# pps-lab/rofl-project-code

Measured on AMD Instinct MI355X. Metric: range-proof elements/sec (create+verify), d=25k 32-bit, higher is better.
Workload: dtype u32x8 (255-bit integer field)

## Files before the change

rofl_project_code_amd/csrc/host_msm.hpp:

```cpp
#pragma once

MsmPlan msm_plan(size_t n, size_t np = 1) {
    MsmPlan p;
    static const size_t t13 = knob("ROFL_MSM_T13") ? (size_t)atol(knob("ROFL_MSM_T13")) : ((size_t)1 << 13);
    static const size_t t10_knob = knob("ROFL_MSM_T10") ? (size_t)atol(knob("ROFL_MSM_T10")) : 0;
    const size_t t10 = t10_knob ? t10_knob : (np >= 32 ? (size_t)1 << 11 : (size_t)1 << 9);
    if (n >= (1u << 17)) p.c = 16; else if (n >= t13) p.c = 13; else if (n >= t10) p.c = 10; else if (n >= 64) p.c = 7; else p.c = 4;
    if (const char *e = knob("ROFL_MSM_C")) { int v = atoi(e); if (v == 4 || v == 7 || v == 10 || v == 13 || v == 16) p.c = (u32)v; }
    p.W = (254 + p.c - 1) / p.c;
    p.W = (253 - p.c + p.c - 1) / p.c + 1;
    p.wide = (253 - p.c) - (p.c - 1) * (p.W - 1);
    p.B = 1u << (p.c - 1);
    p.levels = (p.c - 1) / 3;
    return p;
}
struct MsmOpt { u32 lr_nh = 0, lr_ng = 0; const niels *fb_wtab = nullptr; size_t fb_stride = 0; u32 fb_c = 16; std::function<void()> overlap; std::function<void(size_t)> post; u32 tag = 0;
                std::function<void(size_t, int)> post8;
                const sc *ip_dev = nullptr; u32 ip_nblk = 0; const niels *qpts = nullptr; bool *ip_included = nullptr;
                hipEvent_t pts_ready = nullptr; };

struct MsmAllow { bool fb = true, small = true, two = true, slots = true; };
enum class MsmKind { FixedBase, Small, Slots, CountSort };
struct MsmJob {
    MsmWs *ws = nullptr; size_t np = 0, nq = 0, n = 0, PW = 0; MsmPlan P{}; MsmKind kind = MsmKind::CountSort; bool lr = false, two = false, dev_horner = false;
// ... 157 lines not shown
            u32 best = tile; double best_cost = cost(tile);
            for (u32 t = iter_pts; t < n_side + iter_pts; t += iter_pts) {
                const size_t tiles = (n_side + t - 1) / t;
                if (tiles > 48 || tiles * PW > 4096) continue;
                const double c = cost(t);
                if (c < best_cost * 0.999) { best = t; best_cost = c; }
            }
            if (knob("ROFL_TRACE")) fprintf(stderr, "[rofl] bin_l1 tiling: n_side=%u PW=%zu iter=%u: tile %u (%zu blocks, cost %.0f) -> best %u (%zu blocks, cost %.0f)\n", n_side, PW, iter_pts, tile,
                                            (size_t)((n_side + tile - 1) / tile) * PW, cost(tile), best, (size_t)((n_side + best - 1) / best) * PW, best_cost);
            if (best_cost < 0.85 * cost(tile)) tile = best;
        }
        dim3 grid((n_side + tile - 1) / tile, (u32)PW);
        { KSpan ks(C.tm, st, ROFL_TK_MSM_SCATTER, 0, terms * 32 + terms * P.W * 4);
          ROFL_LAUNCH(k_msm_bin_l1, grid, dim3(1024), (size_t)(tl.nbins + tl.nbins * tl.stage) * 4, st, n_side, tile, iter_pts, mw, mm, d_probs, bcur, bins, btail, tl, d_flag);
          ROFL_LAUNCH(k_msm_bin_l2, dim3(tl.nbins, (u32)PW), dim3(512), (size_t)(2 * 128 * worder_wps + tl.cap_bin) * 4, st, tl, P.B, bcur, bins, (const u32 *)btail, cnt, off, d_flag,
                      worder_wps, worder_shift); }
        ROFL_LAUNCH(k_msm_scan, dim3((unsigned)PW), dim3(P.B >= 1024 ? 1024 : 256), 0, st, P.B, cnt, off, (u32 *)nullptr, perm);
        if (C.tm.enabled) { e0 = C.tm.get(); e1 = C.tm.get(); HIPCHK(hipEventRecord(e0, st)); }
        {
            KSpan ks_acc(C.tm, st, ROFL_TK_MSM_ACCUMULATE_FB, terms * P.W * 7, terms * 32);
            static const char *timeline = knob("ROFL_DBG_ACC_TIMELINE");
            if (timeline) {
                dim3 g = grid1((size_t)Wb * P.B, (u32)nq);
                size_t waves = (size_t)g.x * g.y * (TPB / 64);
                unsigned long long *rec; HIPCHK(hipMalloc(&rec, waves * 32)); HIPCHK(hipMemsetAsync(rec, 0, waves * 32, st));
                ROFL_LAUNCH(k_msm_accumulate_fb_dbg, g, dim3(TPB), 0, st, (u32)n, P.c, Wb, (u32)(np / nq), d_probs, cnt, off, bins, perm, buckets, MSM_LIST_ABS, acc_balance, rec);
                std::vector<unsigned long long> h(waves * 4);
                HIPCHK(hipMemcpyAsync(h.data(), rec, waves * 32, hipMemcpyDeviceToHost, st)); HIPCHK(hipStreamSynchronize(st));
                if (FILE *f = fopen(timeline, "ab")) { unsigned long long hdr[4] = {0x54494d45ull, waves, g.x, g.y}; fwrite(hdr, 8, 4, f); fwrite(h.data(), 8, h.size(), f); fclose(f); }
                HIPCHK(hipFree(rec));
            } else
            ROFL_LAUNCH(k_msm_accumulate_fb, grid1((size_t)Wb * P.B, (u32)nq), dim3(TPB), 0, st, (u32)n, P.c, Wb, (u32)(np / nq), d_probs, cnt, off, bins, perm, buckets, MSM_LIST_ABS,
                        acc_balance | ((worder && nq > 1 && Wb > 1) ? 2u : 0u));
        }
        if (C.tm.enabled) HIPCHK(hipEventRecord(e1, st));
    } else if (J.kind != MsmKind::CountSort) {
        HIPCHK(hipMemsetAsync(cnt, 0, sizeof(u32) * (PW * P.B + 4), st));
        const u32 cap = J.cap;
        u32 *slots = W.sorted.as<u32>(PW * P.B * cap);
        MsmOvf *ovf = W.ovf.as<MsmOvf>(MSM_OVF_MAX);
        u32 *ovf_count = cnt + PW * P.B;
        if (C.msm_lds && n >= C.msm_lds_min && (size_t)P.B * 4 <= 128 * 1024) {
            u32 per_q = fb ? J.sets : P.W;
            u32 tile = n_side;
            u32 wps = fb ? mm.fb_wps : 1;
            while (tile > 1024 && ((size_t)tile * wps > (size_t)C.msm_lds_tile || (size_t)((n_side + tile - 1) / tile) * nq * (lr ? 2 : 1) * per_q < 256)) tile /= 2;
            dim3 grid((n_side + tile - 1) / tile, (u32)(nq * (lr ? 2 : 1) * per_q));
            J.tile = tile;
            uint64_t items = terms * P.W;
            KSpan ks(C.tm, st, ROFL_TK_MSM_SCATTER, 0, terms * 32 + items * 4);
            ROFL_LAUNCH(k_msm_scatter_lds, grid, dim3(1024), (size_t)P.B * 4, st, n_side, tile, mw, mm, d_probs, cnt, slots, cap, ovf_count, ovf, MSM_OVF_MAX);
        } else
            ROFL_LAUNCH(k_msm_scatter_slots, grid1(n, (u32)(nq * P.W)), dim3(TPB), 0, st, (u32)n, mw, mm, d_probs, cnt, slots, cap, ovf_count, ovf, MSM_OVF_MAX);
        ROFL_LAUNCH(k_msm_scan, dim3((unsigned)PW), dim3(P.B >= 1024 ? 1024 : 256), 0, st, P.B, cnt, off, (u32 *)nullptr, perm);
        if (opt.pts_ready) HIPCHK(hipStreamWaitEvent(st, opt.pts_ready, 0));
        if (C.tm.enabled) { e0 = C.tm.get(); e1 = C.tm.get(); HIPCHK(hipEventRecord(e0, st)); }
        {
            uint64_t acc_adds = terms * P.W;
            KSpan ks_acc(C.tm, st, fb ? ROFL_TK_MSM_ACCUMULATE_FB : ROFL_TK_MSM_ACCUMULATE_GEN, acc_adds * 7, terms * 32);
            if (fb) ROFL_LAUNCH(k_msm_accumulate_fb, grid1((size_t)Wb * P.B, (u32)nq), dim3(TPB), 0, st, (u32)n, P.c, Wb, (u32)(np / nq), d_probs, cnt, off, slots, perm, buckets, cap, acc_balance);
            else ROFL_LAUNCH(k_msm_accumulate_gen, grid1((size_t)Wb * P.B, (u32)nq), dim3(TPB), 0, st, (u32)n, P.c, Wb, (u32)(np / nq), d_probs, cnt, off, slots, perm, buckets, cap, acc_balance);
        }
        if (C.tm.enabled) HIPCHK(hipEventRecord(e1, st));
        ROFL_LAUNCH(k_msm_overflow, dim3(1), dim3(64), 0, st, Wb, P.B, (u32)(np / nq), d_probs, ovf_count, ovf, MSM_OVF_MAX, buckets, fb ? 1 : 0);
        HIPCHK(hipMemcpyAsync(h_flag, ovf_count, 4, hipMemcpyDeviceToHost, st));
    } else {
        HIPCHK(hipMemsetAsync(cnt, 0, sizeof(u32) * (PW * P.B + 4), st));
        u32 *sorted = W.sorted.as<u32>(PW * n * 2);
        ROFL_LAUNCH(k_msm_count, grid1(n, (u32)(nq * P.W)), dim3(TPB), 0, st, (u32)n, mw, mm, d_probs, cnt);
        ROFL_LAUNCH(k_msm_scan, dim3((unsigned)PW), dim3(P.B >= 1024 ? 1024 : 256), 0, st, P.B, cnt, off, cur, perm);
        ROFL_LAUNCH(k_msm_scatter, grid1(n, (u32)(nq * P.W)), dim3(TPB), 0, st, (u32)n, mw, mm, d_probs, cur, sorted);
        if (opt.pts_ready) HIPCHK(hipStreamWaitEvent(st, opt.pts_ready, 0));
        if (C.tm.enabled) { e0 = C.tm.get(); e1 = C.tm.get(); HIPCHK(hipEventRecord(e0, st)); }
        ROFL_LAUNCH(k_msm_accumulate_gen, grid1((size_t)Wb * P.B, (u32)nq), dim3(TPB), 0, st, (u32)n, P.c, Wb, (u32)(np / nq), d_probs, cnt, off, sorted, perm, buckets, 0u, acc_balance);
        if (C.tm.enabled) HIPCHK(hipEventRecord(e1, st));
    }
    if (C.tm.enabled) {
        C.tm.acc_ev.push_back({e0, e1}); C.tm.t.msm_accumulate_launches++; C.tm.t.msm_additions += terms * P.W;
        char tg[96]; snprintf(tg, sizeof tg, "msm np=%zu n=%zu c=%u cap=%u fb=%u lr=%d", np, n, P.c, J.kind != MsmKind::CountSort ? J.cap : 0u, fb ? J.sets : 0u, (int)lr); C.tm.acc_tag.push_back(tg);
    }
    const ge *S_in = buckets; const ge *C_in = nullptr;
    u32 E = P.B, nb = 0, lv = 0;
    uint64_t red_adds = 0;
    { u32 e = P.B, b = 0; while (e > 512) { red_adds += (uint64_t)(e / 8) * (11 + 7 * b); e /= 8; b += 3; }
      red_adds += (uint64_t)(e / 8) * (16 + 7 * b); e /= 8; b += 3; while (e > 1) { red_adds += (uint64_t)(e / 2) * (1 + b); e /= 2; b++; } }
    ge *S_fin = J.dev_horner ? W.S[1].as<ge>(PW) : hres_dev;
    ge *C_fin = J.dev_horner ? W.Cacc[1].as<ge>(PW * (size_t)nb_final) : hres_dev + PW;
    {
        KSpan ks_red(C.tm, st, ROFL_TK_MSM_REDUCE, red_adds * PW * 9, (uint64_t)PW * P.B * 128);
        while (E > 512) {
            u32 E8 = E / 8;
            ge *S_out = W.S[lv & 1].as<ge>(PW * E8);
            ge *C_out = W.Cacc[lv & 1].as<ge>(PW * (size_t)(nb + 3) * E8);
            ROFL_LAUNCH(k_msm_reduce_level, grid1((size_t)E8 * (1 + nb), (u32)PW), dim3(TPB), 0, st, E, nb, S_in, C_in, S_out, C_out);
            S_in = S_out; C_in = C_out; E = E8; nb += 3; lv++;
        }
        if (J.dev_horner) { S_fin = W.S[lv & 1].as<ge>(PW); C_fin = W.Cacc[lv & 1].as<ge>(PW * (size_t)nb_final); }
        static const u32 red_fused_max = knob("ROFL_RED_FUSED_T") ? (u32)std::max(64, atoi(knob("ROFL_RED_FUSED_T"))) : 768u;
        u32 fused_items = (E / 8) * (4 + nb), fused_threads = fused_items > 512 ? (fused_items > 640 ? 768 : 640) : fused_items > 256 ? 512 : fused_items > 128 ? 256 : fused_items > 64 ? 128 : 64;
        if (fused_threads > red_fused_max) fused_threads = red_fused_max;
        J.fused_t = fused_threads;
        size_t lds = ((size_t)(E / 8) * (1 + nb + 3) + (size_t)(E / 16) * (1 + nb + 4) + 1) * sizeof(ge);
        ROFL_LAUNCH(k_msm_reduce_fused, dim3((unsigned)PW), dim3(fused_threads), lds, st, E, nb, S_in, C_in, S_fin, C_fin, nb_final);
    }
    if (J.host8)
        ROFL_LAUNCH(k_msm_wsum, grid1(PW * 4), dim3(TPB), 0, st, (u32)PW, (const ge *)S_fin, (const ge *)C_fin, nb_final, hres_dev);
    else if (J.dev_horner)
        ROFL_LAUNCH(k_msm_horner, dim3((unsigned)np), dim3(256), 0, st, mw, (const ge *)S_fin, (const ge *)C_fin, nb_final, hres_dev);
    return J;
}

std::atomic<uint64_t> g_msm_stat[4];
constexpr u32 kMsmTraceMax = 8;
thread_local rofl_msm_attempt_t t_msm_trace[kMsmTraceMax];
thread_local u32 t_msm_trace_n = 0;
bool msm_retry_inner(const MsmJob &J, MsmAllow &al);
bool msm_retry(const MsmJob &J, MsmAllow &al) {
    const bool small = J.kind == MsmKind::Small, two = J.two;
    const bool again = msm_retry_inner(J, al);
    g_msm_stat[again ? (small ? 1 : two ? 2 : 3) : 0].fetch_add(1, std::memory_order_relaxed);
    if (t_msm_trace_n < kMsmTraceMax)
        t_msm_trace[t_msm_trace_n++] = rofl_msm_attempt_t{
            J.fb() ? (uint32_t)ROFL_MSM_FIXED_BASE : small ? (uint32_t)ROFL_MSM_SMALL : J.kind == MsmKind::Slots ? (uint32_t)ROFL_MSM_SLOTS : (uint32_t)ROFL_MSM_COUNT_SORT,
            two ? 1u : 0u, J.P.c, J.P.W, J.cap, J.cap_bin, J.fb() ? J.sets : 0u, small ? J.small_group : 0u,
            J.host8 ? (uint32_t)ROFL_MSM_FIN_HOST8 : J.dev_horner ? (uint32_t)ROFL_MSM_FIN_DEVICE : (uint32_t)ROFL_MSM_FIN_HOST, *J.ws->h_ovf.as<u32>(4), again ? 1u : 0u};
    return again;
}
bool msm_retry_inner(const MsmJob &J, MsmAllow &al) {
    u32 flag = *J.ws->h_ovf.as<u32>(4);
    if (knob("ROFL_TRACE") && J.kind != MsmKind::CountSort)
        fprintf(stderr, "[rofl] msm np=%zu n=%zu c=%u cap=%u fb=%u lr=%d overflow=%u kind=%s two=%d bin=%u tile=%u group=%u fused_t=%u bal=%u horner=%s\n", J.np, J.n, J.P.c, J.cap, J.fb() ? J.sets : 0u, (int)J.lr, flag,
                J.fb() ? "fb" : J.kind == MsmKind::Small ? "small" : "slots", (int)J.two, J.cap_bin, J.tile, J.kind == MsmKind::Small ? J.small_group : 0u, J.fused_t, J.acc_bal, J.host8 ? "host8" : J.dev_horner ? "dev" : "host");
    if (J.kind == MsmKind::Small) { if (flag) { al.small = false; return true; } return false; }
    if (J.two) { if (flag) { al.two = false; return true; } return false; }
    if (J.kind == MsmKind::CountSort) return false;
    if (flag > MSM_OVF_MAX) { if (J.fb()) al.fb = false; else al.slots = false; return true; }
    return false;
}

void msm_finish(Ctx &C, const MsmJob &J, std::vector<ge5> &results, const MsmOpt &opt) {
    const size_t np = J.np, PW = J.PW; const MsmPlan &P = J.P; const u32 sets = J.sets;
    u32 nb = P.c - 1;
    ge *h = J.ws->h_res.as<ge>(PW * (size_t)P.c + np);
    double t0 = now_ms();
    results.resize(np);
    std::vector<double> cpu_each(np, 0.0);
    const char *fin = "host";
    if (J.host8) {
        fin = "host8";
        u32 pos[64];
        for (u32 w = 0; w < P.W; w++) pos[w] = w + 1 == P.W ? 253 - P.c : (w < P.wide ? w * P.c : P.wide * P.c + (w - P.wide) * (P.c - 1));
        C.pool->run((np + 7) / 8, [&](size_t b) {
            double tc0 = now_ms();
            size_t p0 = b * 8; int lanes = (int)std::min<size_t>(8, np - p0);
            ge5 out[8];
            h8::horner8(out, lanes, (int)P.W, pos, [&](int l, int w) { return (const ge *)&h[(p0 + (size_t)l) * P.W + (size_t)w]; });
            for (int l = 0; l < lanes; l++) results[p0 + l] = out[l];
            if (opt.post8) opt.post8(p0, lanes);
            else if (opt.post) for (int l = 0; l < lanes; l++) opt.post(p0 + l);
            cpu_each[p0] = now_ms() - tc0;
        });
    } else if (J.dev_horner) {
        fin = "dev";
        if (opt.post) C.pool->run(np, [&](size_t p) { results[p] = h51::from_ge_loose(h[p]); opt.post(p); });
        else for (size_t p = 0; p < np; p++) results[p] = h51::from_ge_loose(h[p]);
    } else if (J.fb()) {
        auto fb_one = [&](size_t p) {
            size_t base = p * sets;
            ge5 acc = h51::identity(); bool started = false;
            for (int l = (int)nb - 1; l >= 0; l--) {
                if (started) acc = h51::gdouble(acc);
// ... 118 lines not shown
```

rofl_project_code_amd/csrc/host_rt.hpp:

```cpp
#pragma once

struct Knob { const char *name, *dflt, *what; };
static const Knob KNOBS[] = {
    {"ROFL_LANES", "3", "calls that can be in flight on a device (HIP stream + workspace each); 1..16, larger values are clamped (with a note on stderr)"},
    {"ROFL_DEVICES", "0", "option devices: bit mask of the logical devices the batch entry points shard their clients over (0 = the calling thread's device only)"},
    {"ROFL_DEVICE_MAP", "", "logical -> physical HIP device, comma separated (0,0 = two logical devices on GPU 0: how the multi-device paths are tested on a one-GPU box); default: identity"},
    {"ROFL_RCCL_LIB", "librccl.so.1", "the RCCL library rofl_comm_* loads with dlopen (a host that has torch in the process names /opt/rocm/lib/librccl.so.1: the bare soname would resolve to torch's bundled copy)"},
    {"ROFL_HOST_THREADS", "usable cores, in [2, 16]", "threads of the primary lane's host pool (window combination, encodings, transcripts of a round); other lanes: usable cores, in [6, 12]"},
    {"ROFL_POOL_SPIN_US", "400", "how long an idle pool worker polls for the next job before it sleeps (0 = sleep at once)"},
    {"ROFL_BLOCKING_SYNC", "-1", "option blocking_sync: -1 spin while <= 3 calls are in flight, 0 always spin, 1 sleep between polls"},
    {"ROFL_VERIFY_ZIP_TRUNCATE", "0", "option verify_zip_truncate: 1 = the reference's zip-truncating verify_rangeproof"},
    {"ROFL_VERIFY_BATCH", "1", "option verify_batch: 0 = one check per proof, 1 = one per client, 2 = one per batch of clients (bisecting down to per-client checks on failure)"},
    {"ROFL_SIGMA_BATCH", "1", "option sigma_batch: 0 = one check per element in the Sigma-proof verifiers"},
    {"ROFL_STAGE_KEEP_MB", "256", "pinned staging memory a lane keeps between calls (a call that needed more frees it when it ends)"},
    {"ROFL_GENS_LAZY", "1", "0 = the first call of a shape waits for its full fold table (otherwise it is served from the compact table while a background thread builds the full one)"},
    {"ROFL_GENS_LAZY_IDLE_MS", "20", "the background build of a full fold table starts when no call has been in flight for this long (its allocation stalls every HIP call of the process)"},
    {"ROFL_GENS_LAZY_MAX_WAIT_MS", "3000", "... or after this long, whichever comes first (a host that never pauses still gets its full table)"},
    {"ROFL_GENS_RESERVE_MB", "40960", "HBM a table allocation of 4 GB or more leaves free on the device (other contexts / processes / workspaces; the runtime aborts when HBM runs out): the table is narrowed instead"},
    {"ROFL_GENS_BUDGET_MB", "131072", "HBM budget of the generator-table cache (LRU eviction of unpinned entries beyond it)"},
    {"ROFL_FOLD_T1", "3", "IPP rounds before the first generator fold (1..6)"},
    {"ROFL_FOLD_T", "2", "IPP rounds between later folds (1..6)"},
    {"ROFL_FOLD_MIN", "1024", "no fold once fewer generators per chunk would remain (launches with many chunks fold down to 64)"},
    {"ROFL_MSM_BIN_SIGMA", "8", "room of a coarse bin of the two-level sort above twice its mean load, in standard deviations of that load (0 = the fixed 256 entries of rounds 2-3)"},
    {"ROFL_FOLD_TAB", "1", "0 = first fold without the precomputed odd-multiple slices"},
    {"ROFL_FOLD_PB", "32", "piece width of the fold table in bits (16, 32, 64)"},
    {"ROFL_FOLD_W", "10", "NAF width of the fold table (3..10: 2^(w-2) odd multiples per 32-bit piece, 1/(w+1) of the digits non-zero; narrowed until the table fits ROFL_FOLD_TAB_MB)"},
    {"ROFL_FOLD_TAB_MB", "106496", "HBM budget of one (n, m) fold table (cfg 2 at width 10 and cfg 4 at width 9: 102.4 GB of the 288; 57344 = one width less, half the memory, +0.25 ms per cfg-2 proof)"},
    {"ROFL_FOLD_K", "0", "digit-position segments per fold output (1, 2, 4; 0 = by launch size)"},
    {"ROFL_FOLD_THREADS", "131072", "fold launches with fewer threads split their chains into segments"},
    {"ROFL_MSM_FB", "1", "0 = no window tables (every MSM generic)"},
    {"ROFL_MSM_FB_MIN", "4096", "generator sets smaller than this get no window table"},
    {"ROFL_MSM_FB_C", "0", "one window width (13, 15, 16) for every window table; 0 = 16-bit tables, plus a 15-bit one for generator sets below 2^17 that launches with many problems and the verifier use"},
    {"ROFL_MSM_FB_THREADS", "524288", "accumulate threads a fixed-base launch aims for (decides the number of bucket sets)"},
    {"ROFL_MSM_TWO_LEVEL", "1", "0 = slot sort instead of the two-level bucket sort in fixed-base launches"},
    {"ROFL_MSM_SLOTS", "1", "0 = count / scan / scatter sort only (no fixed-capacity structures)"},
    {"ROFL_MSM_LDS", "1", "0 = per-item global atomics instead of LDS ranking in the slot sort"},
    {"ROFL_MSM_LDS_MIN", "8192", "MSMs with fewer terms use the per-item slot sort"},
    {"ROFL_MSM_LDS_TILE", "131072", "items one block of the LDS slot sort ranks"},
    {"ROFL_MSM_SMALL_MAX", "8192", "terms per side up to which a generic MSM runs as one fused launch (0 = off)"},
    {"ROFL_MSM_SMALL_GROUP", "4", "windows of a problem per block of the fused launch at c = 7 with more than 512 bucket arrays (1 = one window per one-wave block, 2, 4)"},
    {"ROFL_MERLIN_X8", "1", "0 = the verifier hashes every chunk's transcript prefix on its own even when the host has AVX-512 (eight chunks per instruction stream otherwise, from 32 chunks on)"},
    {"ROFL_MSM_HOST8", "1", "0 = launches with many problems combine their windows on the device (k_msm_horner) even when the host has AVX-512 IFMA"},
    {"ROFL_MSM_HOST8_MIN", "8", "launches with at least this many problems run their window chains eight per AVX-512 IFMA stream on the host (when the CPU has it)"},
    {"ROFL_MSM_FB_HOST8_MIN", "8", "fixed-base launches with at least this many problems finish eight problems per AVX-512 IFMA task (32 = as in rounds 3-4: one scalar chain per pool task below 32 problems)"},
    {"ROFL_KECCAK_ZMM", "", "host transcripts: 1 = Keccak-f[1600] with one state across five AVX-512 registers, 0 = the scalar rounds; unset = whichever a 50 us measurement at first use finds faster (Intel: the registers, 1.27x; Zen 5: scalar)"},
    {"ROFL_MSM_DEV_HORNER_MIN", "32", "launches with at least this many problems combine their windows on the device"},
    {"ROFL_MSM_T13", "8192", "generic MSMs from this many terms on use 13-bit windows"},
    {"ROFL_MSM_T10", "512 / 2048", "generic MSMs from this many terms on use 10-bit windows (7-bit below, 4-bit below 64); default 2048 for launches with >= 32 problems"},
    {"ROFL_MSM_C", "0", "window width of every generic MSM (4, 7, 10, 13, 16; 0 = by size)"},
    {"ROFL_RED_FUSED_T", "768", "largest block of k_msm_reduce_fused (64 at least: smaller values are raised to one wave)"},
    {"ROFL_ACC_BALANCE", "1", "0 = accumulate blocks in plain descending-load order instead of equal-work blocks"},
    {"ROFL_TRACE", "0", "1 = one line per MSM, window combination, generator fold, table eviction and verifier hashing pass on stderr (which variant ran), 2 = per-phase host timeline of every proof / verification"},
    {"ROFL_DBG_SMALL_TIMELINE", "", "set: per-phase block timings of every fused small-MSM launch on stderr (synchronises; debugging)"},
    {"ROFL_DBG_ACC_TIMELINE", "", "file to append per-wave start / end / placement records of every fixed-base accumulate launch to"},
    {"ROFL_FEMUL_LDS", "0", "rofl_bench_femul: dynamic LDS per block (pins the micro-benchmark's occupancy)"},
    {"ROFL_FEMUL_MODE", "0", "rofl_bench_femul: 0 multiplication chain, 1-3 mixed addition from registers / a 32 KB table / a gathered table"},
    {"ROFL_FEMUL_TABLE", "2097152", "rofl_bench_femul mode 3: table entries (128 B each)"},
};
const char *knob(const char *name) {
#ifndef NDEBUG
    bool known = false; for (const Knob &k : KNOBS) known |= !strcmp(k.name, name);
    if (!known) { fprintf(stderr, "librofl_zk: unregistered knob %s\n", name); abort(); }
#endif
    return getenv(name);
}
static const bool g_keccak_knob_applied = [] { if (const char *e = knob("ROFL_KECCAK_ZMM")) if (*e) keccak_zmm_flag() = atoi(e) != 0 && __builtin_cpu_supports("avx512f"); return true; }();

thread_local std::string g_err;
int fail(int code, const std::string &msg) { g_err = msg; return code; }
std::atomic<uint64_t> g_point_decodes{0};
inline void count_decodes(size_t n) { g_point_decodes.fetch_add((uint64_t)n, std::memory_order_relaxed); }
struct HipErr { hipError_t e; const char *what; };
#define HIPCHK(x) do { hipError_t e__ = (x); if (e__ != hipSuccess) throw HipErr{e__, #x}; } while (0)
#define ROFL_LAUNCH(...) do { (void)hipGetLastError(); hipLaunchKernelGGL(__VA_ARGS__); hipError_t e__ = hipGetLastError(); \
                              if (e__ != hipSuccess && e__ != hipErrorNotReady) throw HipErr{e__, "kernel launch"}; } while (0)

double now_ms() { return std::chrono::duration<double, std::milli>(std::chrono::steady_clock::now().time_since_epoch()).count(); }

sc h_mont(const sc &canon) { return sc_to_mont(canon); }
sc h_canon(const sc &mont) { return sc_from_mont(mont); }
sc h_mul(const sc &a, const sc &b) { return sc_mul_plain(a, b); }
sc h_inv(const sc &canon) { return h_canon(h51::sc_invert_mont_fast(h_mont(canon))); }
bool sc_is_canonical_bytes(const uint8_t *b) { sc s = sc_frombytes(b); return !sc_geq_l(s.v); }

int sc_naf(int8_t out[256], const sc &k) {
    u32 x[9]; for (int i = 0; i < 8; i++) x[i] = k.v[i]; x[8] = 0;
    int top = -1;
    for (int pos = 0; pos < 256; pos++) {
        int d = 0;
        if (x[0] & 1) {
            d = 2 - (int)(x[0] & 3);
            if (d > 0) { x[0] -= 1; }
            else { u64 c = 1; for (int i = 0; i < 9 && c; i++) { c += x[i]; x[i] = (u32)c; c >>= 32; } }
            top = pos;
        }
        out[pos] = (int8_t)d;
        for (int i = 0; i < 8; i++) x[i] = (x[i] >> 1) | (x[i + 1] << 31);
        x[8] >>= 1;
    }
    return top;
}

int wnaf_u64(int16_t out[FOLD_TAB_DIGITS], u64 piece, unsigned w) {
    unsigned __int128 k = piece; int top = -1;
    const int full = 1 << w, half = 1 << (w - 1);
    for (int pos = 0; pos < FOLD_TAB_DIGITS; pos++) {
        int d = 0;
        if (k & 1) { d = (int)(k & (unsigned)(full - 1)); if (d >= half) d -= full; if (d >= 0) k -= (unsigned)d; else k += (unsigned)(-d); top = pos; }
        out[pos] = (int16_t)d; k >>= 1;
    }
    return top;
}

using h51::ge5; using h51::niels5;
struct HostTables { std::vector<niels> B, Bb; std::vector<niels5> B5, Bb5; ge base, bblind; };

void build_fixed_table(std::vector<niels> &tab, ge P) {
    tab.resize(64 * 8);
    for (int w = 0; w < 64; w++) {
        ge acc = P;
        for (int e = 0; e < 8; e++) {
            tab[w * 8 + e] = ge_to_niels(acc);
            acc = ge_add(acc, P);
        }
        for (int k = 0; k < 4; k++) P = ge_double(P);
    }
}
ge5 h_fixed_mul(const std::vector<niels5> &tab, const sc &k_canon) {
    ge5 acc = h51::identity();
    int carry = 0;
    for (int i = 0; i < 64; i++) {
        int v = (int)((k_canon.v[i >> 3] >> ((i & 7) * 4)) & 15) + carry;
        carry = (v + 8) >> 4;
// ... 759 lines not shown
```

rofl_project_code_amd/csrc/kernels.hpp:

```cpp
#pragma once
#include <type_traits>
#include "fe32.hpp"
#include "fe26.hpp"
#include "quad26.hpp"
#include "fd_dbg.hpp"
#include "keccak.hpp"

namespace rofl {

#define TPB 256

#ifndef ROFL_KGROUP
#define ROFL_KGROUP 0
#endif
#define ROFL_KG(g) (ROFL_KGROUP == 0 || ROFL_KGROUP == (g))

typedef unsigned int v4u __attribute__((ext_vector_type(4)));
typedef __attribute__((address_space(1))) v4u g_uint4;
__device__ __forceinline__ niels gload_niels(const niels *p) {
    niels r;
    const g_uint4 *s = (const g_uint4 *)p;
    v4u *d = reinterpret_cast<v4u *>(&r);
#pragma unroll
    for (int i = 0; i < 6; i++) d[i] = s[i];
// ... 1664 lines not shown
        gd acc = gd_add(load_gd(&cs[0]), load_gd(&cs[1]));
#pragma unroll 1
        for (int t = 2; t < 8; t++) acc = gd_add(acc, load_gd(&cs[t]));
        store_gd(&C_out[(size_t)(role - 4) * E8 + g], acc);
        return;
    }
    const ge *s = S_in + (size_t)g * 8;
    if (role == 0) {
        gd acc = gd_add(load_gd(&s[0]), load_gd(&s[1]));
#pragma unroll 1
        for (int t = 2; t < 8; t++) acc = gd_add(acc, load_gd(&s[t]));
        store_gd(&S_out[g], acc);
    } else {
        u32 b = role - 1, st = 1u << b;
        u32 i0 = st, i1 = b == 2 ? 5 : 3, i2 = b == 0 ? 5 : 6, i3 = 7;
        gd acc = gd_add(load_gd(&s[i0]), load_gd(&s[i1]));
        acc = gd_add(acc, load_gd(&s[i2]));
        acc = gd_add(acc, load_gd(&s[i3]));
        store_gd(&C_out[(size_t)(nb + b) * E8 + g], acc);
    }
}
#if ROFL_KG(1)
__global__ void __launch_bounds__(TPB) k_msm_reduce_level(u32 E, u32 nb, const ge *S_in, const ge *C_in, ge *S_out, ge *C_out) {
    u32 pw = blockIdx.y, E8 = E / 8;
    u32 t = blockIdx.x * blockDim.x + threadIdx.x;
    if (t >= E8 * (1 + nb)) return;
    msm_reduce_item(E, nb, S_in + (size_t)pw * E, C_in + (size_t)pw * nb * E, S_out + (size_t)pw * E8, C_out + (size_t)pw * (nb + 3) * E8, t);
}
#endif
__device__ __forceinline__ void msm_binary_level(u32 E, u32 nb, const ge *si, const ge *ci, ge *so, ge *co) {
    const u32 E2 = E / 2, items = E2 * (1 + nb);
    if (items * 4 <= blockDim.x) {
        const u32 item = threadIdx.x >> 2, q = threadIdx.x & 3;
        if (item < items) {
            const u32 role = item / E2, g = item % E2;
            const ge *pa, *pb; ge *dst;
            if (role == 0) { pa = &si[2 * g]; pb = &si[2 * g + 1]; dst = &so[g]; }
            else { const ge *cc = ci + (size_t)(role - 1) * E; pa = &cc[2 * g]; pb = &cc[2 * g + 1]; dst = &co[(size_t)(role - 1) * E2 + g]; }
            const fe fa = reinterpret_cast<const fe *>(pa)[q], fb = reinterpret_cast<const fe *>(pb)[q];
            gq a, b; a.v = fd_unpack(fa); b.v = fd_unpack(fb);
            reinterpret_cast<fe *>(dst)[q] = fd_pack(gq_add(a, b, q).v);
            if (role == 0) reinterpret_cast<fe *>(&co[(size_t)nb * E2 + g])[q] = fb;
        }
        return;
    }
    for (u32 item = threadIdx.x; item < items; item += blockDim.x) {
        u32 role = item / E2, g = item % E2;
        if (role == 0) {
            ge lo = si[2 * g], hi = si[2 * g + 1];
            so[g] = gd_pack(gd_add(gd_unpack(lo), gd_unpack(hi)));
            co[(size_t)nb * E2 + g] = hi;
        } else {
            const ge *cc = ci + (size_t)(role - 1) * E;
            co[(size_t)(role - 1) * E2 + g] = gd_pack(gd_add(gd_unpack(cc[2 * g]), gd_unpack(cc[2 * g + 1])));
        }
    }
}
__device__ __forceinline__ void msm_reduce_fused_body(u32 E, u32 nb, const ge *si, const ge *ci, ge *fin_s, ge *fin_c, unsigned char *smem) {
    ge *buf0 = reinterpret_cast<ge *>(smem);
    u32 E8 = E / 8;
    ge *so = E8 == 1 ? fin_s : buf0, *co = E8 == 1 ? fin_c : buf0 + E8;
    for (u32 item = threadIdx.x; item < E8 * (4 + nb); item += blockDim.x) msm_reduce_item_split(E, nb, si, ci, so, co, item);
    __syncthreads();
    if (E8 == 1) return;
    u32 half = E8 * (1 + nb + 3);
    ge *bufs[2] = {buf0, buf0 + half};
    int sel = 1;
    si = so; ci = co; E = E8; nb += 3;
    while (E > 1) {
        u32 E2 = E / 2;
        if (E2 == 1) { so = fin_s; co = fin_c; } else { so = bufs[sel]; co = bufs[sel] + E2; }
        msm_binary_level(E, nb, si, ci, so, co);
        __syncthreads();
        si = so; ci = co; E = E2; nb += 1; sel ^= 1;
    }
}
#if ROFL_KG(1)
__global__ void __launch_bounds__(768) k_msm_reduce_fused(u32 E, u32 nb, const ge *S_in, const ge *C_in, ge *S_fin, ge *C_fin, u32 nb_final) {
    extern __shared__ __align__(16) unsigned char smem[];
    u32 pw = blockIdx.x;
    msm_reduce_fused_body(E, nb, S_in + (size_t)pw * E, C_in + (size_t)pw * nb * E, S_fin + pw, C_fin + (size_t)pw * nb_final, smem);
}
#endif
__device__ __forceinline__ void msm_reduce_binary_body(u32 E, const ge *si_g, ge *fin_s, ge *fin_c, unsigned char *smem) {
    ge *buf0 = reinterpret_cast<ge *>(smem);
    u32 E2 = E / 2;
    ge *bufs[2] = {buf0, buf0 + (size_t)E2 * 2};
    {
        ge *so = bufs[0], *co = bufs[0] + E2;
        for (u32 g = threadIdx.x; g < E2; g += blockDim.x) {
            ge lo = load_ge(&si_g[2 * g]), hi = load_ge(&si_g[2 * g + 1]);
            so[g] = gd_pack(gd_add(gd_unpack(lo), gd_unpack(hi)));
            co[g] = hi;
        }
    }
    __syncthreads();
    const ge *si = bufs[0], *ci = bufs[0] + E2;
    u32 nb = 1; int sel = 1;
    E = E2;
    while (E > 1) {
        E2 = E / 2;
        ge *so, *co;
        if (E2 == 1) { so = fin_s; co = fin_c; } else { so = bufs[sel]; co = bufs[sel] + E2; }
        msm_binary_level(E, nb, si, ci, so, co);
        __syncthreads();
        si = so; ci = co; E = E2; nb += 1; sel ^= 1;
    }
}
__device__ __forceinline__ void msm_binary_level_inplace(u32 E, u32 nb, ge *buf) {
    const u32 E2 = E / 2, items = E2 * (1 + nb);
    const ge *si = buf, *ci = buf + E;
    if (items * 4 <= blockDim.x) {
        const u32 item = threadIdx.x >> 2, q = threadIdx.x & 3;
        const bool on = item < items;
        const u32 role = on ? item / E2 : 0, g = on ? item % E2 : 0;
        fe res, hi;
        if (on) {
            const ge *pa, *pb;
            if (role == 0) { pa = &si[2 * g]; pb = &si[2 * g + 1]; }
            else { const ge *cc = ci + (size_t)(role - 1) * E; pa = &cc[2 * g]; pb = &cc[2 * g + 1]; }
            const fe fa = reinterpret_cast<const fe *>(pa)[q]; hi = reinterpret_cast<const fe *>(pb)[q];
            gq a, b; a.v = fd_unpack(fa); b.v = fd_unpack(hi);
            res = fd_pack(gq_add(a, b, q).v);
        }
        __syncthreads();
        if (on) {
            ge *so = buf, *co = buf + E2;
            ge *dst = role == 0 ? &so[g] : &co[(size_t)(role - 1) * E2 + g];
            reinterpret_cast<fe *>(dst)[q] = res;
            if (role == 0) reinterpret_cast<fe *>(&co[(size_t)nb * E2 + g])[q] = hi;
        }
        __syncthreads();
        return;
    }
    const u32 item = threadIdx.x;
    const bool on = item < items;
    const u32 role = on ? item / E2 : 0, g = on ? item % E2 : 0;
    ge res, hi;
    if (on) {
        const ge *cc = role == 0 ? si : ci + (size_t)(role - 1) * E;
        const ge lo = cc[2 * g]; hi = cc[2 * g + 1];
        res = gd_pack(gd_add(gd_unpack(lo), gd_unpack(hi)));
    }
    __syncthreads();
    if (on) {
        ge *so = buf, *co = buf + E2;
        if (role == 0) { so[g] = res; co[(size_t)nb * E2 + g] = hi; }
        else co[(size_t)(role - 1) * E2 + g] = res;
    }
    __syncthreads();
}
__device__ __forceinline__ void msm_reduce_binary_multi(u32 E, u32 G, u32 gv, const ge *si_g, ge *fin_s, ge *fin_c, u32 nb_final, unsigned char *smem) {
    ge *buf = reinterpret_cast<ge *>(smem);
    const u32 Et = G * E, E4 = Et / 4;
    {
        const u32 item = threadIdx.x;
        if (item < 3 * E4) {
            const u32 role = item / E4, g = item % E4;
            const u32 tree = (4 * g) / E, in_tree = (4 * g) % E, src_tree = tree < gv ? tree : gv - 1;
            const ge *b = si_g + (size_t)src_tree * E + in_tree;
            const ge x = load_ge(&b[role == 0 ? 0 : role == 1 ? 1 : 2]), y = load_ge(&b[role == 0 ? 1 : 3]);
            buf[(size_t)role * E4 + g] = gd_pack(gd_add(gd_unpack(x), gd_unpack(y)));
        }
        __syncthreads();
        if (4 * E4 <= blockDim.x) {
            const u32 g = threadIdx.x >> 2, q = threadIdx.x & 3;
// ... 1785 lines not shown
```

Before: 1.195 million.

## Replace 8-ary bucket reduction chain with row/column sums and per-bit sums

For bucket arrays of 4096 to 32768 entries, the bucket index is split into row and column bits. The code sums each row and each column, then forms the total and each bit's partial sum from the row or column sums in a second kernel. This swaps the multi-level 8-ary reduction chain plus fused reduce for two launches with fewer additions. The old chain stays available when ROFL_RED_FUSED_T is set.

```diff
diff --git a/rofl_project_code_amd/csrc/host_msm.hpp b/rofl_project_code_amd/csrc/host_msm.hpp
--- a/rofl_project_code_amd/csrc/host_msm.hpp
+++ b/rofl_project_code_amd/csrc/host_msm.hpp
@@ -263,11 +263,19 @@
     const ge *S_in = buckets; const ge *C_in = nullptr;
     u32 E = P.B, nb = 0, lv = 0;
     uint64_t red_adds = 0;
-    { u32 e = P.B, b = 0; while (e > 512) { red_adds += (uint64_t)(e / 8) * (11 + 7 * b); e /= 8; b += 3; }
-      red_adds += (uint64_t)(e / 8) * (16 + 7 * b); e /= 8; b += 3; while (e > 1) { red_adds += (uint64_t)(e / 2) * (1 + b); e /= 2; b++; } }
     ge *S_fin = J.dev_horner ? W.S[1].as<ge>(PW) : hres_dev;
     ge *C_fin = J.dev_horner ? W.Cacc[1].as<ge>(PW * (size_t)nb_final) : hres_dev + PW;
-    {
+    static const bool red_chain = knob("ROFL_RED_FUSED_T") != nullptr;
+    if (!red_chain && P.B >= 4096 && P.B <= 32768) {
+        const u32 lgE = (u32)lg2u((size_t)P.B), k = lgE / 2, rows = 1u << (lgE - k), cols = 1u << k;
+        red_adds = 2 * (uint64_t)P.B - rows - cols + (cols - 1) + (uint64_t)k * (cols / 2 - 1) + (uint64_t)(lgE - k) * (rows / 2 - 1);
+        KSpan ks_red(C.tm, st, ROFL_TK_MSM_REDUCE, red_adds * PW * 9, (uint64_t)PW * P.B * 128);
+        ge *Rs = W.S[0].as<ge>(PW * rows), *Cs = W.Cacc[0].as<ge>(PW * cols);
+        ROFL_LAUNCH(k_msm_rowcol_sums, dim3((rows + cols) / 8, (u32)PW), dim3(256), 0, st, lgE, k, (const ge *)buckets, Rs, Cs);
+        ROFL_LAUNCH(k_msm_bitsums_plain, dim3((unsigned)PW), dim3((1 + lgE) * 32), 0, st, lgE, k, (const ge *)Rs, (const ge *)Cs, S_fin, C_fin, nb_final);
+    } else {
+        { u32 e = P.B, b = 0; while (e > 512) { red_adds += (uint64_t)(e / 8) * (11 + 7 * b); e /= 8; b += 3; }
+          red_adds += (uint64_t)(e / 8) * (16 + 7 * b); e /= 8; b += 3; while (e > 1) { red_adds += (uint64_t)(e / 2) * (1 + b); e /= 2; b++; } }
         KSpan ks_red(C.tm, st, ROFL_TK_MSM_REDUCE, red_adds * PW * 9, (uint64_t)PW * P.B * 128);
         while (E > 512) {
             u32 E8 = E / 8;
diff --git a/rofl_project_code_amd/csrc/host_rt.hpp b/rofl_project_code_amd/csrc/host_rt.hpp
--- a/rofl_project_code_amd/csrc/host_rt.hpp
+++ b/rofl_project_code_amd/csrc/host_rt.hpp
@@ -48,7 +48,7 @@
     {"ROFL_MSM_T13", "8192", "generic MSMs from this many terms on use 13-bit windows"},
     {"ROFL_MSM_T10", "512 / 2048", "generic MSMs from this many terms on use 10-bit windows (7-bit below, 4-bit below 64); default 2048 for launches with >= 32 problems"},
     {"ROFL_MSM_C", "0", "window width of every generic MSM (4, 7, 10, 13, 16; 0 = by size)"},
-    {"ROFL_RED_FUSED_T", "768", "largest block of k_msm_reduce_fused (64 at least: smaller values are raised to one wave)"},
+    {"ROFL_RED_FUSED_T", "768", "largest block of k_msm_reduce_fused (64 at least: smaller values are raised to one wave); when set, arrays of 4096 buckets and more keep the 8-ary chain that ends in that launch instead of the row / column sums"},
     {"ROFL_ACC_BALANCE", "1", "0 = accumulate blocks in plain descending-load order instead of equal-work blocks"},
     {"ROFL_TRACE", "0", "1 = one line per MSM, window combination, generator fold, table eviction and verifier hashing pass on stderr (which variant ran), 2 = per-phase host timeline of every proof / verification"},
     {"ROFL_DBG_SMALL_TIMELINE", "", "set: per-phase block timings of every fused small-MSM launch on stderr (synchronises; debugging)"},
diff --git a/rofl_project_code_amd/csrc/kernels.hpp b/rofl_project_code_amd/csrc/kernels.hpp
--- a/rofl_project_code_amd/csrc/kernels.hpp
+++ b/rofl_project_code_amd/csrc/kernels.hpp
@@ -1770,6 +1770,62 @@
     msm_reduce_fused_body(E, nb, S_in + (size_t)pw * E, C_in + (size_t)pw * nb * E, S_fin + pw, C_fin + (size_t)pw * nb_final, smem);
 }
 #endif
+constexpr u32 RC_T = 32;
+constexpr u32 RC_LDS = RC_T / 2 + RC_T / 4;
+__device__ __forceinline__ void msm_group_sum(const gd &part, u32 t, ge *buf, ge *dst) {
+    ge *A = buf, *B = buf + RC_T / 2;
+    if (t >= RC_T / 2) A[t - RC_T / 2] = gd_pack(part);
+    __syncthreads();
+    if (t < RC_T / 2) A[t] = gd_pack(gd_add(part, gd_unpack(A[t])));
+    __syncthreads();
+    const u32 j = t >> 2, q = t & 3;
+    ge *bufs[2] = {A, B};
+    int sel = 0;
+#pragma unroll
+    for (u32 n = RC_T / 4; n >= 1; n /= 2) {
+        const ge *in = bufs[sel]; ge *out = n == 1 ? dst : &bufs[sel ^ 1][j];
+        if (j < n) {
+            gq a, b; a.v = fd_unpack(reinterpret_cast<const fe *>(&in[2 * j])[q]); b.v = fd_unpack(reinterpret_cast<const fe *>(&in[2 * j + 1])[q]);
+            reinterpret_cast<fe *>(out)[q] = fd_pack(gq_add(a, b, q).v);
+        }
+        if (n > 1) __syncthreads();
+        sel ^= 1;
+    }
+}
+#if ROFL_KG(1)
+__global__ void __launch_bounds__(256, 3) k_msm_rowcol_sums(u32 lgE, u32 k, const ge *buckets, ge *R, ge *C) {
+    __shared__ __align__(16) unsigned char smem[8 * RC_LDS * sizeof(ge)];
+    const u32 pw = blockIdx.y, grp = threadIdx.x / RC_T, t = threadIdx.x % RC_T;
+    const u32 rows = 1u << (lgE - k), cols = 1u << k, g = blockIdx.x * 8 + grp;
+    if (g >= rows + cols) return;
+    const ge *b = buckets + ((size_t)pw << lgE);
+    const bool row = g < rows;
+    const u32 first = row ? g * cols + t : t * cols + (g - rows), stride = row ? RC_T : RC_T * cols, cnt = (row ? cols : rows) / RC_T;
+    gd acc = load_gd(&b[first]);
+#pragma unroll 1
+    for (u32 i = 1; i < cnt; i++) acc = gd_add(acc, load_gd(&b[first + i * stride]));
+    msm_group_sum(acc, t, reinterpret_cast<ge *>(smem) + grp * RC_LDS, row ? R + (size_t)pw * rows + g : C + (size_t)pw * cols + (g - rows));
+}
+__global__ void __launch_bounds__(512) k_msm_bitsums_plain(u32 lgE, u32 k, const ge *R, const ge *C, ge *S_fin, ge *C_fin, u32 nb_final) {
+    __shared__ __align__(16) unsigned char smem[16 * RC_LDS * sizeof(ge)];
+    const u32 pw = blockIdx.x, grp = threadIdx.x / RC_T, t = threadIdx.x % RC_T;
+    const u32 rows = 1u << (lgE - k), cols = 1u << k;
+    const bool all = grp == 0, of_cols = all || grp - 1 < k;
+    const u32 j = all ? 0 : of_cols ? grp - 1 : grp - 1 - k;
+    const ge *src = of_cols ? C + (size_t)pw * cols : R + (size_t)pw * rows;
+    const u32 cnt = (all ? cols : of_cols ? cols / 2 : rows / 2) / RC_T;
+    auto at = [&](u32 m) { return all ? m : ((m >> j) << (j + 1)) | (1u << j) | (m & ((1u << j) - 1)); };
+    gd acc = load_gd(src + at(t));
+    ge nx = load_ge(src + at(cnt > 1 ? t + RC_T : t));
+#pragma unroll 1
+    for (u32 i = 1; i < cnt; i++) {
+        const gd p = gd_unpack(nx);
+        nx = load_ge(src + at(i + 1 < cnt ? t + (i + 1) * RC_T : t));
+        acc = gd_add(acc, p);
+    }
+    msm_group_sum(acc, t, reinterpret_cast<ge *>(smem) + grp * RC_LDS, all ? S_fin + pw : C_fin + (size_t)pw * nb_final + (grp - 1));
+}
+#endif
 __device__ __forceinline__ void msm_reduce_binary_body(u32 E, const ge *si_g, ge *fin_s, ge *fin_c, unsigned char *smem) {
     ge *buf0 = reinterpret_cast<ge *>(smem);
     u32 E2 = E / 2;
```

After: 1.215 million (median of 4 runs). 1.7% higher.
